# radiocosmology/draco

Measured on AMD Instinct MI355X. Metric: m-modes/sec through MModeTransform+DirtyMapMaker (128-feed, 256-freq), higher is better.
Workload: dtype f64 accumulate; B stored complex128; FFT complex64 (as the reference); 1 GPU; cfg3: 128-feed (379 stacked baselines), 256 freq per GPU (256 in the job), 1024 RA, lmax=mmax=512: MModeTransform.process + DirtyMapMaker.process through the task classes (131328 (m,f) solves + alm2map to nside=256 IQUV maps per GPU and day); parallelism=freq-sharded x1, weak scaling (no collective in the timed region)

## Files before the change

### draco_amd/csrc/dmm_ctx.hip

```cpp
#include <stdio.h>
#include <string.h>

#include "dmm_internal.h"

static thread_local char g_err[512] = "";

int dmm_set_error(int code, const char* fmt, ...) {
  va_list ap;
  va_start(ap, fmt);
  vsnprintf(g_err, sizeof(g_err), fmt, ap);
  va_end(ap);
  return code;
}

static const char* const kProfNames[DMM_PROF_NSLOT] = {"gram", "chol", "tridiag", "ql", "backproj", "band", "chase", "solve", "null"};

static void prof_collect(dmm_ctx* c) {
  for (dmm_prof_span& sp : c->prof_open) {
    float ms = 0.f;
    if (hipEventSynchronize(sp.b) == hipSuccess && hipEventElapsedTime(&ms, sp.a, sp.b) == hipSuccess) {
      c->prof_us[sp.slot] += 1e3 * (double)ms;
      ++c->prof_n[sp.slot];
    }
    (void)hipEventDestroy(sp.a);
// ... 105 lines not shown
  else if (!strcmp(name, "ml_rank_stop")) c->opt_ml_rank_stop = (int)value;
  else if (!strcmp(name, "ml_chase_split")) c->opt_ml_chase_split = (int)value;
  else if (!strcmp(name, "dirty_prio")) c->opt_dirty_prio = (int)value;
  else if (!strcmp(name, "ml_eigen")) c->opt_ml_eigen = (int)value;
  else if (!strcmp(name, "ringmap_variant")) c->opt_ringmap_variant = (int)value;
  else if (!strcmp(name, "ml_reduce")) c->opt_ml_reduce = (int)value;
  else if (!strcmp(name, "gram_stage")) c->opt_gram_stage = (int)value;
  else if (!strcmp(name, "wiener_overlap")) c->opt_wiener_overlap = (int)value;
  else if (!strcmp(name, "ml_workspace_mib")) c->opt_ml_ws_mib = value > 0 ? value : 0;
  else if (!strcmp(name, "regrid_workspace_mib")) c->opt_regrid_ws_mib = value > 0 ? value : 0;
  else if (!strcmp(name, "wiener_workspace_mib")) c->opt_wiener_ws_mib = value > 0 ? value : 0;
  else if (!strcmp(name, "profile")) {
    prof_collect(c);
    for (int k = 0; k < DMM_PROF_NSLOT; ++k) c->prof_us[k] = 0.0, c->prof_n[k] = 0;
    c->opt_profile = value != 0;
  }
  else return dmm_set_error(DMM_E_ARG, "dmm_ctx_set_option: unknown option '%s'", name);
  return DMM_OK;
}

int dmm_ctx_get_counter(dmm_ctx* c, const char* name, int64_t* value) {
  DMM_REQUIRE(c != nullptr && name != nullptr && value != nullptr, "dmm_ctx_get_counter: NULL argument");
  if (!strcmp(name, "ml_tiles_direct")) *value = c->ml_tiles_direct;
  else if (!strcmp(name, "ml_tiles_eigen")) *value = c->ml_tiles_eigen;
  else if (!strcmp(name, "ml_tiles_null")) *value = c->ml_tiles_null;
  else if (!strcmp(name, "ml_tiles_stopped")) *value = c->ml_tiles_stopped;
  else if (!strcmp(name, "ml_gram_cached")) *value = c->ml_gram_cached;
  else if (!strcmp(name, "ml_tiles_basis")) *value = c->ml_tiles_basis;
  else if (!strcmp(name, "ml_stop_cols")) *value = c->ml_stop_cols;
  else if (!strcmp(name, "ml_gram_flops")) *value = c->ml_gram_flops;
  else if (!strcmp(name, "ml_band_bytes")) *value = c->ml_band_bytes;
  else if (!strcmp(name, "ml_tiles_ql_failed")) *value = c->ml_tiles_ql_failed;
  else if (!strcmp(name, "ml_early_chunks")) *value = c->ml_early_chunks;
  else if (!strcmp(name, "ml_two_stage_max_order")) *value = dmm_ml_two_stage_max_order();
  else if (!strcmp(name, "build_ab")) {
#ifdef DMM_AB
    *value = 1;
#else
    *value = 0;
#endif
  }
  else if (!strcmp(name, "opt_ml_eigen")) *value = c->opt_ml_eigen;
  else if (!strcmp(name, "opt_sht_synth_form")) *value = c->opt_sht_synth_form;
  else if (!strncmp(name, "prof_", 5)) {
    const size_t len = strlen(name);
    const bool want_n = len > 7 && !strcmp(name + len - 2, "_n");
    const bool want_us = len > 8 && !strcmp(name + len - 3, "_us");
    int slot = -1;
    for (int k = 0; k < DMM_PROF_NSLOT; ++k) {
      const size_t nl = strlen(kProfNames[k]);
      if (!strncmp(name + 5, kProfNames[k], nl) && name[5 + nl] == '_' && 5 + nl + (want_n ? 2 : 3) == len) slot = k;
    }
    if (slot < 0 || !(want_n || want_us)) return dmm_set_error(DMM_E_ARG, "dmm_ctx_get_counter: unknown counter '%s'", name);
    prof_collect(c);
    *value = want_n ? c->prof_n[slot] : (int64_t)(c->prof_us[slot] + 0.5);
  }
  else return dmm_set_error(DMM_E_ARG, "dmm_ctx_get_counter: unknown counter '%s'", name);
  return DMM_OK;
}

int dmm_ctx_set_ml_basis(dmm_ctx* c, void* U, double* sigma, int32_t* rank, int64_t nslots, int rmax, int build) {
  DMM_REQUIRE(c != nullptr, "dmm_ctx_set_ml_basis: ctx is NULL");
  DMM_REQUIRE(U == nullptr || (sigma != nullptr && rank != nullptr && nslots > 0 && rmax >= 64 && rmax % 64 == 0),
              "dmm_ctx_set_ml_basis: a basis needs sigma, rank, a slot count and rmax a multiple of 64");
  c->ml_bs_U = (double2*)U;
  c->ml_bs_sigma = U ? sigma : nullptr;
// ... 65 lines not shown
```

### draco_amd/csrc/dmm_internal.h

```cpp
#pragma once
#include <hip/hip_runtime.h>
#include <stdint.h>
#include <stdarg.h>
#include <map>
#include <vector>

#include "draco_amd.h"

template <typename T2>
struct dmm_fft_tables {
  int n = 0;
  int M = 0;
  T2* tw = nullptr;
  T2* chirp = nullptr;
  T2* bfilt = nullptr;
};

enum dmm_prof_slot { DMM_PROF_GRAM = 0, DMM_PROF_CHOL, DMM_PROF_TRIDIAG, DMM_PROF_QL, DMM_PROF_BACKPROJ, DMM_PROF_BAND, DMM_PROF_CHASE, DMM_PROF_SOLVE, DMM_PROF_NULL, DMM_PROF_NSLOT };
struct dmm_prof_span {
  hipEvent_t a, b;
  int slot;
};

struct dmm_ctx {
  int device = 0;
  hipStream_t stream = nullptr;
  hipEvent_t ev0 = nullptr, ev1 = nullptr;
  hipStream_t aux_stream = nullptr;
  hipStream_t aux_stream_b = nullptr;
  hipEvent_t aux_ev[4] = {nullptr, nullptr, nullptr, nullptr};
  int* aux_pinned = nullptr;
  size_t aux_pinned_n = 0;
  int num_cu = 256;
  std::map<int, dmm_fft_tables<float2>> fft_f32;
  std::map<int, dmm_fft_tables<double2>> fft_f64;
  std::map<int64_t, void*> sht;
  int opt_dirty_variant = 0;
  int opt_grid_mult = 0;
  int opt_dirty_prio = 0;
  int opt_dirty_static = 0;
  int opt_dirty_nofill = 0;
  int opt_project_grid_mult = 0;
  int opt_project_variant = 0;
  int opt_ml_inner_sweeps = 0, opt_ml_outer_sweeps = 0;
  int opt_sht_variant = 0;
  int opt_sht_synth_form = 0;
  int opt_ml_eigen = 0;
  int64_t opt_regrid_ws_mib = 0;
  int64_t opt_ml_ws_mib = 0, opt_wiener_ws_mib = 0;
  int opt_ml_shortcut = 0;
  int ml_probe_every = 8;
  double ml_pass_rate = 1.0;
  int opt_ml_null = 0;
  int64_t ml_gram_flops = 0, ml_band_bytes = 0;
  int64_t ml_tiles_null = 0;
  int opt_ml_chase_split = 0;
  int opt_ml_rank_stop = 0;
  int64_t ml_order_hist[17] = {};
  int64_t ml_tiles_stopped = 0, ml_stop_cols = 0;
  int64_t ml_tiles_direct = 0, ml_tiles_eigen = 0;
  int64_t ml_tiles_ql_failed = 0;
  int opt_ringmap_variant = 0;
  int opt_wiener_overlap = 1;
  int opt_gram_stage = 0;
  int opt_ml_reduce = 0;
  double2* ml_bs_U = nullptr;
  double* ml_bs_sigma = nullptr;
  int32_t* ml_bs_rank = nullptr;
  int64_t ml_bs_slots = 0;
// ... 125 lines not shown
```

### draco_amd/csrc/sht.hip

```cpp
#include "sht_common.h"
#include "sht_legendre.h"
#include "sht_rings.h"

namespace {

int get_geom(dmm_ctx* ctx, int nside, int lmax, int mmax, ShtGeom* out) {
  const int64_t key = ((int64_t)nside << 40) | ((int64_t)lmax << 20) | (int64_t)mmax;
  auto it = ctx->sht.find(key);
  const int nring = 4 * nside - 1;
  const size_t nd = (size_t)3 * nring + (mmax + 1);
  const size_t bytes = nd * sizeof(double) + (size_t)nring * sizeof(int64_t) + (size_t)nring * sizeof(int);
  const size_t coef_ofs = (bytes + 63) / 64 * 64;
  const size_t coef_rows = (size_t)coef_row0(mmax + 1, lmax);
  int blue_rmax = 0;
  std::vector<int64_t> bf_off(1, 0);
  int64_t bf_total = 0;
  for (int ir = 1; ir < nside && blue_len(ir) <= kMaxBlue; ++ir) {
    bf_off.push_back(bf_total);
    bf_total += blue_len(ir);
    blue_rmax = ir;
  }
  const size_t bfo_ofs = coef_ofs + coef_rows * sizeof(Coef);
  const size_t bf_ofs = (bfo_ofs + bf_off.size() * sizeof(int64_t) + 63) / 64 * 64;
  const size_t phase_ofs = (bf_ofs + (size_t)bf_total * sizeof(double2) + 63) / 64 * 64;
  int tw_len = kMaxBlue;
  while (tw_len < 4 * nside) tw_len <<= 1;
  const size_t tw_ofs = phase_ofs + (size_t)nring * (mmax + 1) * sizeof(double2);
  const size_t chirp_ofs = tw_ofs + (size_t)(tw_len / 2) * sizeof(double2);
  const size_t total = chirp_ofs + (size_t)2 * blue_rmax * (blue_rmax + 1) * sizeof(double2);
  if (it == ctx->sht.end()) {
    std::vector<unsigned char> h(bytes);
    double* z = reinterpret_cast<double*>(h.data());
    double* sth = z + nring;
    double* phi0 = sth + nring;
    double* lfac = phi0 + nring;
    int64_t* start = reinterpret_cast<int64_t*>(lfac + (mmax + 1));
    int* nphi = reinterpret_cast<int*>(start + nring);
    const int64_t npix = 12LL * nside * nside, ncap = 2LL * nside * (nside - 1);
    for (int k = 0; k < nring; ++k) {
      const int64_t ir = k + 1;
      if (ir < nside) {
        z[k] = 1.0 - (double)(ir * ir) / (3.0 * nside * (double)nside);
        nphi[k] = (int)(4 * ir);
        phi0[k] = M_PI / (4.0 * ir);
        start[k] = 2 * ir * (ir - 1);
      } else if (ir <= 3LL * nside) {
        z[k] = (2.0 * nside - ir) * 2.0 / (3.0 * nside);
        nphi[k] = 4 * nside;
        phi0[k] = ((ir - nside + 1) & 1) * M_PI / (4.0 * nside);
        start[k] = ncap + (ir - nside) * 4LL * nside;
      } else {
        const int64_t ip = 4LL * nside - ir;
        z[k] = -(1.0 - (double)(ip * ip) / (3.0 * nside * (double)nside));
        nphi[k] = (int)(4 * ip);
        phi0[k] = M_PI / (4.0 * ip);
        start[k] = npix - 2 * ip * (ip + 1);
      }
      sth[k] = sqrt((1.0 - z[k]) * (1.0 + z[k]));
    }
    double acc = 0.5 * (log2(1.0) - log2(4.0 * M_PI));
    lfac[0] = acc;
    double prod = 0.0;
    for (int m = 1; m <= mmax; ++m) {
      prod += log2((2.0 * m - 1.0) / (2.0 * m));
      lfac[m] = 0.5 * (log2(2.0 * m + 1.0) - log2(4.0 * M_PI) + prod);
    }
    void* d = nullptr;
    DMM_HIP(hipMalloc(&d, total));
    unsigned char* db = static_cast<unsigned char*>(d);
    hipError_t e = hipMemcpy(d, h.data(), bytes, hipMemcpyHostToDevice);
    if (e == hipSuccess) e = hipMemcpy(db + bfo_ofs, bf_off.data(), bf_off.size() * sizeof(int64_t), hipMemcpyHostToDevice);
    if (e == hipSuccess) {
      hipLaunchKernelGGL(k_fill_coef, dim3(mmax + 1), dim3(256), 0, ctx->stream, reinterpret_cast<Coef*>(db + coef_ofs), lmax);
      e = hipGetLastError();
    }
    if (e == hipSuccess && blue_rmax > 0) {
      const int Mmax = blue_len(blue_rmax);
      const size_t lds = ((size_t)Mmax + 1 + Mmax / 2) * sizeof(double2);
      e = hipFuncSetAttribute((const void*)k_build_bfilt, hipFuncAttributeMaxDynamicSharedMemorySize, (int)lds);
      if (e == hipSuccess) {
        hipLaunchKernelGGL(k_build_bfilt, dim3(blue_rmax), dim3(kFftThreads), lds, ctx->stream,
                           reinterpret_cast<double2*>(db + bf_ofs), reinterpret_cast<const int64_t*>(db + bfo_ofs));
        e = hipGetLastError();
      }
    }
    if (e == hipSuccess) {
      hipLaunchKernelGGL(k_fill_ring_tables, dim3(nring + 1 + blue_rmax), dim3(256), 0, ctx->stream,
                         reinterpret_cast<const double*>(db) + 2 * (size_t)nring , nring, mmax,
                         reinterpret_cast<double2*>(db + phase_ofs), reinterpret_cast<double2*>(db + tw_ofs), tw_len,
                         reinterpret_cast<double2*>(db + chirp_ofs));
      e = hipGetLastError();
    }
    if (e != hipSuccess) {
      (void)hipFree(d);
      return dmm_set_error((int)e, "sht geometry upload: %s", hipGetErrorString(e));
    }
    it = ctx->sht.emplace(key, d).first;
  }
  ShtGeom g;
  g.nside = nside;
  g.lmax = lmax;
  g.mmax = mmax;
  g.nring = nring;
  g.block = it->second;
  g.z = reinterpret_cast<double*>(g.block);
  g.sth = g.z + nring;
  g.phi0 = g.sth + nring;
  g.lfac = g.phi0 + nring;
  g.start = reinterpret_cast<int64_t*>(g.lfac + (mmax + 1));
  g.nphi = reinterpret_cast<int*>(g.start + nring);
  unsigned char* gb = static_cast<unsigned char*>(g.block);
  g.coef = reinterpret_cast<double*>(gb + coef_ofs);
  g.bf_off = reinterpret_cast<int64_t*>(gb + bfo_ofs);
  g.bfilt = reinterpret_cast<double2*>(gb + bf_ofs);
  g.blue_rmax = blue_rmax;
  g.phase = reinterpret_cast<double2*>(gb + phase_ofs);
  g.tw = reinterpret_cast<double2*>(gb + tw_ofs);
  g.tw_len = tw_len;
  g.chirp = reinterpret_cast<double2*>(gb + chirp_ofs);
  *out = g;
  return DMM_OK;
}

int check_args(const char* who, dmm_ctx* ctx, const void* a, const void* b, int nfreq, int npol, int lmax, int mmax,
               int nside) {
  DMM_REQUIRE(ctx && a && b, "%s: NULL argument", who);
  DMM_REQUIRE(nfreq >= 1 && lmax >= 0 && mmax >= 0 && mmax <= lmax, "%s: bad sizes nfreq=%d lmax=%d mmax=%d", who, nfreq, lmax, mmax);
  DMM_REQUIRE(npol == 1 || npol == 4, "%s: npol must be 1 or 4 (got %d)", who, npol);
  DMM_REQUIRE(nside >= 1 && (nside & (nside - 1)) == 0 && nside <= 8192, "%s: nside must be a power of two (got %d)", who, nside);
  return DMM_OK;
}

size_t chunk_freqs(int nfreq, int npol, int nring, int mmax) {
  const size_t grp = npol == 4 ? kSynF : 1;
  const size_t per_f = (size_t)npol * nring * (mmax + 1) * sizeof(double2);
  size_t nf = ((size_t)1 << 30) / per_f / grp * grp;
  if (nf < grp) nf = grp;
  if (nf > (size_t)nfreq) nf = nfreq;
  const size_t nchunk = ((size_t)nfreq + nf - 1) / nf;
  const size_t c = ((size_t)nfreq + nchunk - 1) / nchunk;
  return c < (size_t)nfreq ? (c + grp - 1) / grp * grp : c;
}

size_t coef_scratch_bytes(size_t nfc, int npol, int nring, int mmax) {
  const size_t nfs = npol == 4 ? (nfc + kSynF - 1) / kSynF * kSynF : nfc;
  return nfs * npol * nring * (size_t)(mmax + 1) * sizeof(double2);
}

struct ClassLaunch {
  RingClass rc;
  int nblock;
  int nphi_max;
  bool blue;
};

std::vector<ClassLaunch> ring_classes(const ShtGeom& g) {
  std::vector<ClassLaunch> out;
  ClassLaunch b;
  b.rc.belt = 1;
  b.rc.r_lo = b.rc.r_hi = 0;
  b.rc.M = 4 * g.nside;
  b.rc.logM = 0;
  while ((1 << b.rc.logM) < b.rc.M) ++b.rc.logM;
  b.nblock = 2 * g.nside + 1;
  b.nphi_max = 4 * g.nside;
  b.blue = false;
  out.push_back(b);
  for (int ir = 1; ir < g.nside;) {
    const int M = blue_len(ir);
    int hi = ir;
    while (hi + 1 < g.nside && blue_len(hi + 1) == M) ++hi;
    ClassLaunch c;
    c.rc.belt = 0;
    c.rc.r_lo = ir;
    c.rc.r_hi = hi;
    c.rc.M = M;
    c.rc.logM = 0;
    while ((1 << c.rc.logM) < M) ++c.rc.logM;
    c.nblock = 2 * (hi - ir + 1);
    c.nphi_max = 4 * hi;
    c.blue = true;
    out.push_back(c);
    ir = hi + 1;
  }
  return out;
}

size_t ring_fft_lds(const ShtGeom& g, const ClassLaunch& c, int nrow, int force_direct) {
  if (force_direct) return 0;
  if (c.blue && c.rc.r_hi > g.blue_rmax) return 0;
  const size_t lds = ((size_t)nrow * (c.rc.M + 1) + c.rc.M / 2 + (c.blue ? c.nphi_max : 0)) * sizeof(double2);
  return lds <= 160 * 1024 ? lds : 0;
}

size_t ring_synth_lds(const ShtGeom& g, const ClassLaunch& c, int nb, bool stage_all, int force_direct) {
  if (force_direct) return 0;
  if (c.blue && c.rc.r_hi > g.blue_rmax) return 0;
  const int nm = g.mmax + 1;
  const bool staged = stage_all || 4 * (c.blue ? c.rc.r_lo : g.nside) < nm;
  const size_t lds = ((size_t)nb * (c.rc.M + 1) + c.rc.M / 2 + (c.blue ? c.nphi_max : 0) + (staged ? (size_t)nb * 2 * nm : 0)) *
                     sizeof(double2);
  return lds <= 160 * 1024 ? lds : 0;
}

using RingKernel = void (*)(RingParams, RingClass);

int launch_ring(RingKernel kern, dim3 grid, int threads, size_t lds, hipStream_t st, const RingParams& rp, const RingClass& rc) {
  if (lds > 160 * 1024) return dmm_set_error(DMM_E_UNSUPPORTED, "SHT ring stage needs %zu bytes of LDS (nside too large)", lds);
  DMM_HIP(hipFuncSetAttribute((const void*)kern, hipFuncAttributeMaxDynamicSharedMemorySize, (int)lds));
  hipLaunchKernelGGL(kern, grid, dim3(threads), lds, st, rp, rc);
  DMM_HIP(hipGetLastError());
  return DMM_OK;
}

RingParams ring_params(const ShtGeom& g, int nf, int npol, double2* b, double* map, const double* map_ref) {
  RingParams rp;
  rp.g = g;
  rp.nf = nf;
  rp.npol = npol;
  rp.b = b;
  rp.map = map;
  rp.map_ref = map_ref;
  rp.npix = 12LL * g.nside * g.nside;
  rp.stage_all = 0;
  return rp;
}

#define DMM_BY_NPOL(npol, f, ...) ((npol) == 4 ? f<4>(__VA_ARGS__) : f<1>(__VA_ARGS__))

template <int NPOL>
int synth_chunk(dmm_ctx* ctx, const ShtGeom& g, const double2* alm, int n_m, int nf, double2* b, double* map) {
  LegParams lp;
  lp.g = g;
  lp.nf = nf;
  lp.npol = NPOL;
  lp.n_m = n_m;
  lp.alm = alm;
  lp.b = b;
  if (NPOL == 4 && !(ctx->opt_sht_variant & 8)) {
    const int npair = (g.nring + 1) / 2;
    const int nrc = (npair + kThreads - 1) / kThreads;
    const int nx = g.mmax + 1;
    const int64_t col_bytes = (int64_t)4 * n_m * (g.lmax + 1) * (int64_t)sizeof(double2);
    const bool fits8 = 2 * kLegF * col_bytes < ((int64_t)1 << 32), fits4 = kLegF * col_bytes < ((int64_t)1 << 32);
    if ((ctx->opt_sht_variant & 64) || ctx->opt_sht_synth_form == 1 || !fits4) {
      const int nz = (nf + kLegF - 1) / kLegF;
      hipLaunchKernelGGL(k_leg_synth_mfma, dim3(nx, nrc, nz), dim3(kThreads), 0, ctx->stream, lp);
    } else if ((ctx->opt_sht_variant & 128) || !fits8) {
      const int nz = (nf + kLegF - 1) / kLegF;
      hipLaunchKernelGGL(k_leg_synth_mfma2<1>, dim3(nx, nrc, nz), dim3(kThreads), 0, ctx->stream, lp);
    } else {
      const int nz = (nf + 2 * kLegF - 1) / (2 * kLegF);
      hipLaunchKernelGGL(k_leg_synth_mfma2<2>, dim3(nx, nrc, nz), dim3(kThreads), 0, ctx->stream, lp);
    }
  } else {
    hipLaunchKernelGGL(k_leg_synth<NPOL>, dim3(g.mmax + 1, nf), dim3(kThreads), 0, ctx->stream, lp);
  }
  DMM_HIP(hipGetLastError());
  RingParams rp = ring_params(g, nf, NPOL, b, map, nullptr);
  constexpr int KF = NPOL == 4 ? kSynF : 1;
  const dim3 per_ring((nf + KF - 1) / KF, NPOL == 4 ? 2 : 1);
  const int force_direct = ctx->opt_sht_variant & 4;
  constexpr int N2 = NPOL == 4 ? 2 : 1, N4 = NPOL == 4 ? 4 : 1;
  static const RingKernel fft_kernel[3][2] = {{k_ring_synth_fft<NPOL, 1, false>, k_ring_synth_fft<NPOL, 1, true>},
                                              {k_ring_synth_fft<NPOL, N2, false>, k_ring_synth_fft<NPOL, N2, true>},
                                              {k_ring_synth_fft<NPOL, N4, false>, k_ring_synth_fft<NPOL, N4, true>}};
  for (const ClassLaunch& c : ring_classes(g)) {
    int nb = 0;
    size_t lds = 0;
    rp.stage_all = 0;
    for (int tier = 0; tier < 3 && nb == 0; ++tier)
      for (int b = KF; b >= 1 && nb == 0; b >>= 1) {
        const size_t l = ring_synth_lds(g, c, b, tier == 0, force_direct);
        if (l != 0 && l <= (tier < 2 ? (size_t)80 * 1024 : (size_t)160 * 1024)) nb = b, lds = l, rp.stage_all = tier == 0;
      }
    const int rc = nb == 0 ? launch_ring(k_ring_synth<NPOL>, dim3(c.nblock, nf), kThreads, (size_t)NPOL * (g.mmax + 1) * sizeof(double2),
                                         ctx->stream, rp, c.rc)
                           : launch_ring(fft_kernel[nb >> 1][c.blue], dim3(c.nblock, per_ring.x, per_ring.y), kFftThreads, lds,
                                         ctx->stream, rp, c.rc);
    if (rc) return rc;
  }
  return DMM_OK;
}

template <int NPOL>
int anal_chunk(dmm_ctx* ctx, const ShtGeom& g, const double* map, int n_m, int nf, double2* b, double2* alm, int accumulate,
               const double* map_ref = nullptr) {
  const RingParams rp = ring_params(g, nf, NPOL, b, const_cast<double*>(map), map_ref);
  constexpr int NROWS = NPOL == 4 ? 2 : 1;
  const int force_direct = ctx->opt_sht_variant & 4;
  static const RingKernel fft_kernel[2][2] = {{k_ring_anal_fft<NPOL, 1, false>, k_ring_anal_fft<NPOL, 1, true>},
                                              {k_ring_anal_fft<NPOL, NROWS, false>, k_ring_anal_fft<NPOL, NROWS, true>}};
  for (const ClassLaunch& c : ring_classes(g)) {
    const size_t lds2 = ring_fft_lds(g, c, NROWS, force_direct), lds1 = ring_fft_lds(g, c, 1, force_direct);
    const bool both = NROWS == 2 && lds2 != 0 && lds2 <= 80 * 1024;
    const int rc = lds1 == 0 ? launch_ring(k_ring_anal<NPOL>, dim3(c.nblock, nf), kThreads, (size_t)NPOL * c.nphi_max * sizeof(double),
                                           ctx->stream, rp, c.rc)
                             : launch_ring(fft_kernel[both][c.blue], dim3(c.nblock, nf, both ? 1 : NROWS), kFftThreads,
                                           both ? lds2 : lds1, ctx->stream, rp, c.rc);
    if (rc) return rc;
  }
  LegAnalParams lp;
  lp.g = g;
  lp.nf = nf;
  lp.npol = NPOL;
  lp.n_m = n_m;
  lp.b = b;
  lp.alm = alm;
  lp.accumulate = accumulate;
  if (NPOL == 4 && !(ctx->opt_sht_variant & 8)) {
    hipLaunchKernelGGL(k_leg_anal_mfma, dim3(g.mmax + 1, (nf + kLegF - 1) / kLegF), dim3(kThreads), 0, ctx->stream, lp);
    DMM_HIP(hipGetLastError());
    return DMM_OK;
  }
  constexpr int NV = NPOL == 4 ? 8 : 2;
  const size_t lds2 = (size_t)(g.lmax + 1) * NV * sizeof(double) + (size_t)2 * (kThreads / 64) * kAnalBatch * NV * sizeof(double);
  DMM_HIP(hipFuncSetAttribute((const void*)k_leg_anal<NPOL>, hipFuncAttributeMaxDynamicSharedMemorySize, (int)lds2));
  hipLaunchKernelGGL(k_leg_anal<NPOL>, dim3(g.mmax + 1, nf), dim3(kThreads), lds2, ctx->stream, lp);
  DMM_HIP(hipGetLastError());
  return DMM_OK;
}

}

extern "C" {

int dmm_alm2map(dmm_ctx* ctx, const void* alm, int nfreq, int npol, int lmax, int mmax, int nside, double* map) {
  int rc = check_args("dmm_alm2map", ctx, alm, map, nfreq, npol, lmax, mmax, nside);
  if (rc) return rc;
  DMM_HIP(hipSetDevice(ctx->device));
  ShtGeom g;
  rc = get_geom(ctx, nside, lmax, mmax, &g);
  if (rc) return rc;
  const size_t nfc = chunk_freqs(nfreq, npol, g.nring, mmax);
  void* scratch = nullptr;
  rc = dmm_get_scratch(ctx, coef_scratch_bytes(nfc, npol, g.nring, mmax), &scratch);
  if (rc) return rc;
  const int64_t npix = 12LL * nside * nside;
  const int n_m = mmax + 1;
  for (int f0 = 0; f0 < nfreq; f0 += (int)nfc) {
    const int nf = (int)((size_t)(nfreq - f0) < nfc ? (size_t)(nfreq - f0) : nfc);
    const double2* a = (const double2*)alm + (int64_t)f0 * npol * n_m * (lmax + 1);
    double* mp = map + (int64_t)f0 * npol * npix;
    rc = DMM_BY_NPOL(npol, synth_chunk, ctx, g, a, n_m, nf, (double2*)scratch, mp);
    if (rc) return rc;
  }
  return DMM_OK;
}

int dmm_map2alm(dmm_ctx* ctx, const double* map, int nfreq, int npol, int lmax, int mmax, int nside, int niter,
                void* alm) {
  int rc = check_args("dmm_map2alm", ctx, map, alm, nfreq, npol, lmax, mmax, nside);
  if (rc) return rc;
  DMM_REQUIRE(niter >= 0 && niter <= 64, "dmm_map2alm: niter=%d out of range", niter);
  if ((size_t)npol * 4 * nside * sizeof(double) > 150 * 1024)
    return dmm_set_error(DMM_E_UNSUPPORTED, "dmm_map2alm: nside=%d too large for the in-LDS ring stage", nside);
  DMM_HIP(hipSetDevice(ctx->device));
  ShtGeom g;
  rc = get_geom(ctx, nside, lmax, mmax, &g);
  if (rc) return rc;
  const int64_t npix = 12LL * nside * nside;
  size_t nfc = chunk_freqs(nfreq, npol, g.nring, mmax);
  const size_t b_bytes = coef_scratch_bytes(nfc, npol, g.nring, mmax);
  const size_t r_bytes = niter > 0 ? nfc * npol * (size_t)npix * sizeof(double) : 0;
  void* scratch = nullptr;
  rc = dmm_get_scratch(ctx, b_bytes + r_bytes, &scratch);
  if (rc) return rc;
  double2* b = (double2*)scratch;
  double* resid = (double*)((unsigned char*)scratch + b_bytes);
  const int n_m = mmax + 1;
  for (int f0 = 0; f0 < nfreq; f0 += (int)nfc) {
    const int nf = (int)((size_t)(nfreq - f0) < nfc ? (size_t)(nfreq - f0) : nfc);
    double2* a = (double2*)alm + (int64_t)f0 * npol * n_m * (lmax + 1);
    const double* mp = map + (int64_t)f0 * npol * npix;
    rc = DMM_BY_NPOL(npol, anal_chunk, ctx, g, mp, n_m, nf, b, a, 0);
    if (rc) return rc;
    for (int it = 0; it < niter; ++it) {
      rc = DMM_BY_NPOL(npol, synth_chunk, ctx, g, a, n_m, nf, b, resid);
      if (rc) return rc;
      rc = DMM_BY_NPOL(npol, anal_chunk, ctx, g, resid, n_m, nf, b, a, 1, mp);
      if (rc) return rc;
    }
  }
  return DMM_OK;
}

}
```

### draco_amd/csrc/sht_common.h

```cpp
#pragma once
#include <math.h>

#include <vector>

#include "dmm_internal.h"
#include "fft_lds.h"

namespace {


constexpr int kThreads = 256;
constexpr double kBig = 0x1p+740, kSmallStep = 0x1p-800;

constexpr int kSynF = 4;
constexpr int kSynRow = kSynF * 4;
__host__ __device__ __forceinline__ int64_t syn4_at(int f, int m, int ring, int r, int nring, int nm) {
  return ((((int64_t)(f / kSynF) * 2 + r) * nring + ring) * nm + m) * kSynRow + 4 * (f % kSynF);
}
__host__ __device__ __forceinline__ int syn4_slot(int pol) { return pol == 1 || pol == 2 ? 1 : 0; }

struct ShtGeom {
  int nside, lmax, mmax, nring;
  double* z;
  double* sth;
  double* phi0;
  int* nphi;
  int64_t* start;
  double* lfac;
  double* coef;
  double2* bfilt;
  int64_t* bf_off;
  int blue_rmax;
  double2* phase;
  double2* tw;
  int tw_len;
  double2* chirp;
  void* block;
};

__host__ __device__ __forceinline__ int64_t coef_row0(int m, int lmax) {
  return (int64_t)m * (lmax + 1) - (int64_t)m * (m - 1) / 2;
}

struct LegParams {
  ShtGeom g;
  int nf;
  int npol;
  int n_m;
  const double2* alm;
  double2* b;
};

struct Coef {
  double ra, rb;
  double c1, c2;
  double cd, c3;
  double c4, pad;
};

typedef const __attribute__((address_space(4))) double* kptr;
// ... 20 lines not shown
    Coef q;
    const double dl = (double)l, dm = (double)m;
    const double A = sqrt((dl * dl - dm * dm) / (4.0 * dl * dl - 1.0));
    const double l1 = dl - 1.0;
    const double Ap = (l > m) ? sqrt((l1 * l1 - dm * dm) / (4.0 * l1 * l1 - 1.0)) : 0.0;
    q.ra = (l > m) ? 1.0 / A : 0.0;
    q.rb = (l > m) ? Ap / A : 0.0;
    const double c = (l >= 2) ? 2.0 / sqrt((dl - 1.0) * dl * (dl + 1.0) * (dl + 2.0)) : 0.0;
    const double d = (l >= 1) ? sqrt((2.0 * dl + 1.0) / (2.0 * dl - 1.0) * (dl * dl - dm * dm)) : 0.0;
    q.c1 = c * (dl - dm * dm);
    q.c2 = c * 0.5 * dl * (dl - 1.0);
    q.cd = c * d;
    q.c3 = c * dm * (dl - 1.0);
    q.c4 = c * dm * d;
    q.pad = 0.0;
    coef[l - m] = q;
  }
}
static_assert(sizeof(Coef) == 64, "Coef row");

__device__ __forceinline__ void lam_start(double lfac_m, int m, double sth, double& v, int& nsc) {
  const double lg = lfac_m + (double)m * log2(sth);
  nsc = 0;
  if (lg < -700.0) nsc = (int)ceil((-lg - 700.0) / 800.0);
  v = exp2(lg + 800.0 * (double)nsc);
  if (m & 1) v = -v;
}

__device__ __forceinline__ bool ring_skips_m(int m, int lmax, double sth) {
  const double ofs = fmax(100.0, 0.01 * (double)lmax);
  return (double)m > (double)lmax * sth + ofs + 2.0;
}

}
```

### draco_amd/csrc/sht_legendre.h

```cpp
#pragma once
#include "sht_common.h"

namespace {

typedef double v4d __attribute__((ext_vector_type(4)));

struct LegRing {
  double x, inv_s2, xs2, lam, lam_prev;
  int nsc;
};

__device__ __forceinline__ LegRing leg_ring_start(const ShtGeom& g, int m, int r, int npair) {
  LegRing R = {0.0, 0.0, 0.0, 0.0, 0.0, -1};
  if (r < npair) {
    const double sth = g.sth[r];
    R.x = g.z[r];
    R.inv_s2 = 1.0 / (sth * sth);
    R.xs2 = R.x * R.inv_s2;
    if (!ring_skips_m(m, g.lmax, sth)) lam_start(g.lfac[m], m, sth, R.lam, R.nsc);
  }
  return R;
}

__device__ __forceinline__ void leg_advance(LegRing& R, double ra, double rb) {
// ... 103 lines not shown
      const int kc = k < nl ? k : nl - 1;
      __builtin_amdgcn_s_waitcnt(0xc07f);
      Ops o;
      o.q = load_coef(coef + 8 * kc);
      o.aT = load_c(a[0] + 2 * kc);
      o.aE = o.aB = o.aV = make_double2(0.0, 0.0);
      if (NPOL == 4) {
        o.aE = load_c(a[NPOL > 1 ? 1 : 0] + 2 * kc);
        o.aB = load_c(a[NPOL > 1 ? 2 : 0] + 2 * kc);
        o.aV = load_c(a[NPOL > 1 ? 3 : 0] + 2 * kc);
      }
      return o;
    };
    Ops cur = fetch(0);
    for (int k = 0; k < nl; k += 2) {
      Ops nxt = fetch(k + 1);
#pragma unroll
      for (int t = 0; t < NR; ++t) step(R[t], S[t], cur.q, cur.aT, cur.aE, cur.aB, cur.aV, k == 0, true);
      if (k + 1 >= nl) break;
      cur = fetch(k + 2);
#pragma unroll
      for (int t = 0; t < NR; ++t) step(R[t], S[t], nxt.q, nxt.aT, nxt.aE, nxt.aB, nxt.aV, false, false);
    }
#pragma unroll
    for (int t = 0; t < NR; ++t) {
      const int r = r0 + t * kThreads + threadIdx.x;
      if (r >= npair) continue;
      const int rs = nring - 1 - r;
      const Sums& g = S[t];
      auto val = [&](double2 s, double2 an, double sgn) { return make_double2(s.x + sgn * an.x, s.y + sgn * an.y); };
      if (NPOL == 1) {
        p.b[((int64_t)f * nring + r) * mstride + m] = val(g.Ts, g.Ta, 1.0);
        if (rs != r) p.b[((int64_t)f * nring + rs) * mstride + m] = val(g.Ts, g.Ta, -1.0);
      } else {
        double* bout = reinterpret_cast<double*>(p.b);
        auto put = [&](int ring, int tr, double2 v0, double2 v1) {
          double* q = bout + syn4_at(f, m, ring, tr, nring, (int)mstride);
          *reinterpret_cast<double2*>(q) = make_double2(v0.x, v1.x);
          *reinterpret_cast<double2*>(q + 2) = make_double2(v0.y, v1.y);
        };
        put(r, 0, val(g.Ts, g.Ta, 1.0), val(g.Qs, g.Qa, 1.0));
        put(r, 1, val(g.Vs, g.Va, 1.0), val(g.Us, g.Ua, 1.0));
        if (rs != r) {
          put(rs, 0, val(g.Ts, g.Ta, -1.0), val(g.Qs, g.Qa, -1.0));
          put(rs, 1, val(g.Vs, g.Va, -1.0), val(g.Us, g.Ua, -1.0));
        }
      }
    }
  }
}

constexpr int kLegL = 8, kLegF = 4, kLegPitch = 72;
static_assert(kLegF == kSynF, "a frequency group of the MFMA columns is one group of the synthesis scratch");

template <class TileRing>
__device__ __forceinline__ void leg_store_syn4(const LegParams& p, int f, int m, const LegCol& col, int kq, const v4d (&acc)[4][4],
                                               TileRing tile0) {
  const int nring = p.g.nring, npair = (nring + 1) / 2, nm = p.g.mmax + 1;
  double* bout = reinterpret_cast<double*>(p.b) + 2 * col.comp;
#pragma unroll
  for (int t = 0; t < 4; ++t)
#pragma unroll
    for (int reg = 0; reg < 4; ++reg) {
      const int rr = tile0(t) + kq + 4 * reg;
      if (rr >= npair) continue;
      const int rs = nring - 1 - rr;
      const double tv = acc[t][0][reg], tva = acc[t][1][reg], qu = acc[t][2][reg], qua = acc[t][3][reg];
      *reinterpret_cast<double2*>(bout + syn4_at(f, m, rr, col.c >> 1, nring, nm)) = make_double2(tv + tva, qu + qua);
      if (rs != rr) *reinterpret_cast<double2*>(bout + syn4_at(f, m, rs, col.c >> 1, nring, nm)) = make_double2(tv - tva, qu - qua);
    }
}

__global__ __launch_bounds__(kThreads, 2) void k_leg_synth_mfma(LegParams p) {
  __shared__ double slab[kThreads / 64][3][kLegL][kLegPitch];
  const int m = blockIdx.x, rc = blockIdx.y, f0 = blockIdx.z * kLegF;
  const int lmax = p.g.lmax, nl = lmax - m + 1;
  const int lane = threadIdx.x & 63, wave = threadIdx.x >> 6;
  double(*sl)[kLegL][kLegPitch] = slab[wave];

  LegRing R = leg_ring_start(p.g, m, rc * kThreads + threadIdx.x, (p.g.nring + 1) / 2);
  const bool wave_live = __any(R.nsc >= 0);

  const int li = lane & 15, kq = lane >> 4;
  const LegCol col = leg_col(lane);
  const int f = f0 + col.fi;
  const bool fok = f < p.nf;
  auto colptr = [&](int pol, int comp) {
    return reinterpret_cast<const double*>(p.alm + (((int64_t)(fok ? f : 0) * 4 + pol) * p.n_m + m) * (lmax + 1) + m) + comp;
  };
  const double* pTV = colptr(col.polTV, col.comp);
  const double* p1 = colptr(col.pol1, col.comp);
  const double* p2 = colptr(col.pol2, col.comp ^ 1);
  const double s2 = col.f2neg ? -1.0 : 1.0;

  v4d acc[4][4];
#pragma unroll
  for (int t = 0; t < 4; ++t)
#pragma unroll
// ... 563 lines not shown
```

### draco_amd/csrc/sht_rings.h

```cpp
#pragma once
#include "sht_common.h"

namespace {

struct RingParams {
  ShtGeom g;
  int nf, npol;
  double2* b;
  double* map;
  int64_t npix;
  const double* map_ref;
  int stage_all;
};

struct RingClass {
  int belt;
  int r_lo, r_hi;
  int M, logM;
};
constexpr int kMinBlue = 256, kMaxBlue = 4096;

__host__ __device__ __forceinline__ int blue_len(int ir) {
  int M = kMinBlue;
  while (M < 8 * ir - 1) M <<= 1;
  return M;
}

__device__ __forceinline__ int class_ring(const RingClass& rc, const ShtGeom& g, int i) {
  if (rc.belt) return g.nside - 1 + i;
  const int ir = rc.r_lo + (i >> 1);
  return (i & 1) ? g.nring - ir : ir - 1;
}

template <int NPOL>
__global__ __launch_bounds__(kThreads) void k_ring_synth(RingParams p, RingClass rc) {
  extern __shared__ __align__(16) unsigned char smem[];
  double2* c = reinterpret_cast<double2*>(smem);
  const int ring = class_ring(rc, p.g, blockIdx.x);
  const int f = blockIdx.y;
  const int nm = p.g.mmax + 1;
  const double phi0 = p.g.phi0[ring];
  const int nphi = p.g.nphi[ring];
  for (int idx = threadIdx.x; idx < NPOL * nm; idx += kThreads) {
    const int pol = idx / nm, m = idx - pol * nm;
    double2 v;
    if (NPOL == 1) {
      v = p.b[((int64_t)f * p.g.nring + ring) * nm + m];
    } else {
      const double* q = reinterpret_cast<const double*>(p.b) + syn4_at(f, m, ring, pol >> 1, p.g.nring, nm) + syn4_slot(pol);
      v = make_double2(q[0], q[2]);
    }
    double sn, cs;
    sincos((double)m * phi0, &sn, &cs);
    const double fac = m == 0 ? 1.0 : 2.0;
    c[idx] = make_double2(fac * (v.x * cs - v.y * sn), fac * (v.x * sn + v.y * cs));
  }
  __syncthreads();
  const int64_t base = p.g.start[ring];
  for (int j = threadIdx.x; j < nphi; j += kThreads) {
    double sn, cs;
    sincospi(2.0 * (double)j / (double)nphi, &sn, &cs);
    double pr = 1.0, pi_ = 0.0;
    double acc[NPOL];
#pragma unroll
    for (int q = 0; q < NPOL; ++q) acc[q] = 0.0;
    for (int m = 0; m < nm; ++m) {
#pragma unroll
      for (int q = 0; q < NPOL; ++q) {
        const double2 cm = c[q * nm + m];
        acc[q] = fma(cm.x, pr, fma(-cm.y, pi_, acc[q]));
      }
      const double nr = pr * cs - pi_ * sn;
      pi_ = fma(pr, sn, pi_ * cs);
      pr = nr;
    }
#pragma unroll
    for (int q = 0; q < NPOL; ++q) p.map[((int64_t)f * NPOL + q) * p.npix + base + j] = acc[q];
  }
}

constexpr int kFftThreads = 256;

struct RingLds {
  dmm_fft::C<double>* buf;
  dmm_fft::C<double>* tw;
  dmm_fft::C<double>* chirp;
};

template <int NROW, bool BLUE>
__device__ __forceinline__ RingLds ring_lds(unsigned char* smem, const ShtGeom& g, int N, int M) {
  RingLds l;
  l.buf = reinterpret_cast<dmm_fft::C<double>*>(smem);
  l.tw = l.buf + NROW * (M + 1);
  l.chirp = l.tw + (M >> 1);
  const int stride = g.tw_len / M;
  for (int k = threadIdx.x; k < (M >> 1); k += kFftThreads) {
    const double2 t = g.tw[k * stride];
    l.tw[k] = {t.x, t.y};
  }
// ... 42 lines not shown
  if (BLUE) dmm_fft::bluestein_convolve<double, kFftThreads>(l.buf, l.tw, bfilt, NROW, M, logM, P, true);
  else dmm_fft::fft_dif8<double, kFftThreads>(l.buf, l.tw, NROW, M, logM, P);
}

template <bool BLUE>
__device__ __forceinline__ dmm_fft::C<double> ring_dft_at(const RingLds& l, int r, int k, int M, int logM) {
  if (BLUE) return dmm_fft::cmul<double>(l.buf[r * (M + 1) + k], l.chirp[k]);
  return l.buf[r * (M + 1) + dmm_fft::bitrev(k, logM)];
}

template <int NPOL, int NB, bool BLUE>
__global__ __launch_bounds__(kFftThreads) void k_ring_synth_fft(RingParams p, RingClass rc) {
  using dmm_fft::C;
  constexpr int KF = NPOL == 4 ? kSynF : 1;
  static_assert(KF % NB == 0, "passes of NB transforms");
  extern __shared__ __align__(16) unsigned char smem[];
  const int ring = class_ring(rc, p.g, blockIdx.x), r = NPOL == 4 ? (int)blockIdx.z : 0;
  const int f0 = KF * blockIdx.y, nfb = min(KF, p.nf - f0);
  const int n = p.g.nphi[ring], M = rc.M, P = M + 1;
  const RingLds l = ring_lds<NB, BLUE>(smem, p.g, n, M);
  if (BLUE) __syncthreads();
  const int nm = p.g.mmax + 1;
  const double2* phase = p.g.phase + (int64_t)ring * nm;
  auto load = [&](int fi, int m, double2& va, double2& vb) {
    if (NPOL == 1) {
      va = p.b[((int64_t)(f0 + fi) * p.g.nring + ring) * nm + m];
    } else {
      const double* q = reinterpret_cast<const double*>(p.b) + syn4_at(f0 + fi, m, ring, r, p.g.nring, nm);
      const double2 re = *reinterpret_cast<const double2*>(q), im = *reinterpret_cast<const double2*>(q + 2);
      va = r == 0 ? make_double2(re.x, im.x) : make_double2(re.y, im.y);
      vb = r == 0 ? make_double2(re.y, im.y) : make_double2(re.x, im.x);
    }
  };
  const bool staged = p.stage_all || n < nm;
  C<double>* rot = l.chirp + (BLUE ? 4 * rc.r_hi : 0);
  const double2* bfilt = BLUE ? p.g.bfilt + p.g.bf_off[rc.belt ? 0 : rc.r_lo + ((int)blockIdx.x >> 1)] : nullptr;
  const int64_t base = p.g.start[ring];
  for (int fb = 0; fb < nfb; fb += NB) {
    if (fb > 0) __syncthreads();
    if (staged) {
      for (int q = threadIdx.x; q < NB * nm; q += kFftThreads) {
        const int m = q / NB, j = q - m * NB;
        C<double> a = {0.0, 0.0}, b = {0.0, 0.0};
        if (fb + j < nfb) {
          const double2 ph = phase[m];
          const double cs = ph.x, sn = ph.y;
          double2 va, vb;
          load(fb + j, m, va, vb);
          a = {va.x * cs - va.y * sn, va.x * sn + va.y * cs};
          if (NPOL == 4) b = {vb.x * cs - vb.y * sn, vb.x * sn + vb.y * cs};
          if (m == 0) a.y = b.y = 0.0;
        }
        rot[(j * 2 + 0) * nm + m] = a;
        rot[(j * 2 + 1) * nm + m] = b;
      }
      __syncthreads();
    }
    for (int k = threadIdx.x; k < M; k += kFftThreads) {
      double zr[NB], zi[NB];
#pragma unroll
      for (int j = 0; j < NB; ++j) zr[j] = zi[j] = 0.0;
      if (k < n && staged) {
        for (int m = k; m < nm; m += n) {
#pragma unroll
          for (int j = 0; j < NB; ++j) {
            const C<double> a = rot[(j * 2 + 0) * nm + m], b = rot[(j * 2 + 1) * nm + m];
            zr[j] += a.x - b.y;
            zi[j] += a.y + b.x;
          }
        }
        for (int m = (k == 0 ? n : n - k); m < nm; m += n) {
#pragma unroll
          for (int j = 0; j < NB; ++j) {
            const C<double> a = rot[(j * 2 + 0) * nm + m], b = rot[(j * 2 + 1) * nm + m];
            zr[j] += a.x + b.y;
            zi[j] += b.x - a.y;
          }
        }
      } else if (k < n) {
        for (int m = k; m < nm; m += n) {
          const double2 ph = phase[m];
          const double cs = ph.x, sn = ph.y;
#pragma unroll
          for (int j = 0; j < NB; ++j) {
            if (fb + j >= nfb) continue;
            double2 va, vb;
            load(fb + j, m, va, vb);
            double ar = va.x * cs - va.y * sn, ai = va.x * sn + va.y * cs;
            double br = 0.0, bi = 0.0;
            if (NPOL == 4) {
              br = vb.x * cs - vb.y * sn;
              bi = vb.x * sn + vb.y * cs;
            }
            if (m == 0) ai = bi = 0.0;
            zr[j] += ar - bi;
            zi[j] += ai + br;
          }
        }
        for (int m = (k == 0 ? n : n - k); m < nm; m += n) {
          const double2 ph = phase[m];
          const double cs = ph.x, sn = ph.y;
#pragma unroll
          for (int j = 0; j < NB; ++j) {
            if (fb + j >= nfb) continue;
            double2 va, vb;
            load(fb + j, m, va, vb);
            const double ar = va.x * cs - va.y * sn, ai = va.x * sn + va.y * cs;
            double br = 0.0, bi = 0.0;
            if (NPOL == 4) {
              br = vb.x * cs - vb.y * sn;
              bi = vb.x * sn + vb.y * cs;
            }
            zr[j] += ar + bi;
            zi[j] += br - ai;
          }
        }
      }
#pragma unroll
      for (int j = 0; j < NB; ++j) {
        C<double> v = {zr[j], -zi[j]};
        if (BLUE && k < n) v = dmm_fft::cmul<double>(v, l.chirp[k]);
        l.buf[j * P + k] = v;
      }
    }
    __syncthreads();
    ring_dft<NB, BLUE>(l, bfilt, M, rc.logM);
    for (int j = threadIdx.x; j < n; j += kFftThreads) {
#pragma unroll
      for (int jj = 0; jj < NB; ++jj) {
        if (fb + jj >= nfb) continue;
        const int64_t f = f0 + fb + jj;
        const C<double> y = ring_dft_at<BLUE>(l, jj, j, M, rc.logM);
// ... 131 lines not shown
```

Before: 2070 m-modes/s.

## Truncate per-ring m range in SHT synthesis using precomputed mlim table

Computes a per-ring maximum m (mlim) on the device from the existing ring_skips_m criterion, caches it per geometry, and uses it to bound the Legendre output writes, the ring synthesis loops and the staged rotation buffer. Polar rings where high m contribute negligibly then skip the loads, rotations and fold-ins for those m. LDS for the staged buffer is sized by the per-class max nrot, which may let more blocks fit per CU. Adds a one-time device sync and counters, and relies on the Legendre stage leaving unwritten slots unused.

```diff
diff --git a/draco_amd/csrc/dmm_ctx.hip b/draco_amd/csrc/dmm_ctx.hip
--- a/draco_amd/csrc/dmm_ctx.hip
+++ b/draco_amd/csrc/dmm_ctx.hip
@@ -161,6 +161,8 @@
   else if (!strcmp(name, "ml_band_bytes")) *value = c->ml_band_bytes;
   else if (!strcmp(name, "ml_tiles_ql_failed")) *value = c->ml_tiles_ql_failed;
   else if (!strcmp(name, "ml_early_chunks")) *value = c->ml_early_chunks;
+  else if (!strcmp(name, "sht_skipped_slots")) *value = c->sht_skipped_slots;
+  else if (!strcmp(name, "sht_mlim_mismatch")) *value = c->sht_mlim_mismatch;
   else if (!strcmp(name, "ml_two_stage_max_order")) *value = dmm_ml_two_stage_max_order();
   else if (!strcmp(name, "build_ab")) {
 #ifdef DMM_AB
diff --git a/draco_amd/csrc/dmm_internal.h b/draco_amd/csrc/dmm_internal.h
--- a/draco_amd/csrc/dmm_internal.h
+++ b/draco_amd/csrc/dmm_internal.h
@@ -35,6 +35,8 @@
   std::map<int, dmm_fft_tables<float2>> fft_f32;
   std::map<int, dmm_fft_tables<double2>> fft_f64;
   std::map<int64_t, void*> sht;
+  std::map<int64_t, std::vector<int>> sht_mlim;
+  int64_t sht_skipped_slots = 0, sht_mlim_mismatch = 0;
   int opt_dirty_variant = 0;
   int opt_grid_mult = 0;
   int opt_dirty_prio = 0;
diff --git a/draco_amd/csrc/sht.hip b/draco_amd/csrc/sht.hip
--- a/draco_amd/csrc/sht.hip
+++ b/draco_amd/csrc/sht.hip
@@ -1,15 +1,17 @@
+#include <algorithm>
+
 #include "sht_common.h"
 #include "sht_legendre.h"
 #include "sht_rings.h"
 
 namespace {
 
-int get_geom(dmm_ctx* ctx, int nside, int lmax, int mmax, ShtGeom* out) {
+int get_geom(dmm_ctx* ctx, int nside, int lmax, int mmax, ShtGeom* out, const int** mlim_host) {
   const int64_t key = ((int64_t)nside << 40) | ((int64_t)lmax << 20) | (int64_t)mmax;
   auto it = ctx->sht.find(key);
   const int nring = 4 * nside - 1;
   const size_t nd = (size_t)3 * nring + (mmax + 1);
-  const size_t bytes = nd * sizeof(double) + (size_t)nring * sizeof(int64_t) + (size_t)nring * sizeof(int);
+  const size_t bytes = nd * sizeof(double) + (size_t)nring * sizeof(int64_t) + 2 * sizeof(unsigned long long) + (size_t)2 * nring * sizeof(int);
   const size_t coef_ofs = (bytes + 63) / 64 * 64;
   const size_t coef_rows = (size_t)coef_row0(mmax + 1, lmax);
   int blue_rmax = 0;
@@ -35,7 +37,7 @@
     double* phi0 = sth + nring;
     double* lfac = phi0 + nring;
     int64_t* start = reinterpret_cast<int64_t*>(lfac + (mmax + 1));
-    int* nphi = reinterpret_cast<int*>(start + nring);
+    int* nphi = reinterpret_cast<int*>(start + nring + 2);
     const int64_t npix = 12LL * nside * nside, ncap = 2LL * nside * (nside - 1);
     for (int k = 0; k < nring; ++k) {
       const int64_t ir = k + 1;
@@ -91,10 +93,25 @@
                          reinterpret_cast<double2*>(db + chirp_ofs));
       e = hipGetLastError();
     }
+    std::vector<int> mlim_h(nring);
+    unsigned long long stats[2] = {0, 0};
+    if (e == hipSuccess) {
+      unsigned long long* dstats = reinterpret_cast<unsigned long long*>(db + nd * sizeof(double) + (size_t)nring * sizeof(int64_t));
+      int* dmlim = reinterpret_cast<int*>(dstats + 2) + nring;
+      hipLaunchKernelGGL(k_fill_mlim, dim3(nring), dim3(256), 0, ctx->stream, reinterpret_cast<const double*>(db) + nring , lmax,
+                         mmax, dmlim, dstats);
+      e = hipGetLastError();
+      if (e == hipSuccess) e = hipMemcpyAsync(mlim_h.data(), dmlim, (size_t)nring * sizeof(int), hipMemcpyDeviceToHost, ctx->stream);
+      if (e == hipSuccess) e = hipMemcpyAsync(stats, dstats, sizeof(stats), hipMemcpyDeviceToHost, ctx->stream);
+      if (e == hipSuccess) e = hipStreamSynchronize(ctx->stream);
+    }
     if (e != hipSuccess) {
       (void)hipFree(d);
       return dmm_set_error((int)e, "sht geometry upload: %s", hipGetErrorString(e));
     }
+    ctx->sht_skipped_slots += (int64_t)stats[0];
+    ctx->sht_mlim_mismatch += (int64_t)stats[1];
+    ctx->sht_mlim[key] = std::move(mlim_h);
     it = ctx->sht.emplace(key, d).first;
   }
   ShtGeom g;
@@ -108,7 +125,9 @@
   g.phi0 = g.sth + nring;
   g.lfac = g.phi0 + nring;
   g.start = reinterpret_cast<int64_t*>(g.lfac + (mmax + 1));
-  g.nphi = reinterpret_cast<int*>(g.start + nring);
+  g.nphi = reinterpret_cast<int*>(g.start + nring + 2);
+  g.mlim = g.nphi + nring;
+  *mlim_host = ctx->sht_mlim[key].data();
   unsigned char* gb = static_cast<unsigned char*>(g.block);
   g.coef = reinterpret_cast<double*>(gb + coef_ofs);
   g.bf_off = reinterpret_cast<int64_t*>(gb + bfo_ofs);
@@ -154,8 +173,13 @@
   bool blue;
 };
 
-std::vector<ClassLaunch> ring_classes(const ShtGeom& g) {
+std::vector<ClassLaunch> ring_classes(const ShtGeom& g, const int* mlim = nullptr) {
   std::vector<ClassLaunch> out;
+  auto nrot_of = [&](int first, int last) {
+    int v = 0;
+    for (int k = first; mlim && k <= last; ++k) v = std::max(v, std::max(mlim[k], mlim[g.nring - 1 - k]) + 1);
+    return v;
+  };
   ClassLaunch b;
   b.rc.belt = 1;
   b.rc.r_lo = b.rc.r_hi = 0;
@@ -165,6 +189,7 @@
   b.nblock = 2 * g.nside + 1;
   b.nphi_max = 4 * g.nside;
   b.blue = false;
+  b.rc.nrot = nrot_of(g.nside - 1, 2 * g.nside - 1);
   out.push_back(b);
   for (int ir = 1; ir < g.nside;) {
     const int M = blue_len(ir);
@@ -180,6 +205,7 @@
     c.nblock = 2 * (hi - ir + 1);
     c.nphi_max = 4 * hi;
     c.blue = true;
+    c.rc.nrot = nrot_of(ir - 1, hi - 1);
     out.push_back(c);
     ir = hi + 1;
   }
@@ -193,12 +219,12 @@
   return lds <= 160 * 1024 ? lds : 0;
 }
 
-size_t ring_synth_lds(const ShtGeom& g, const ClassLaunch& c, int nb, bool stage_all, int force_direct) {
+size_t ring_synth_lds(const ShtGeom& g, const ClassLaunch& c, int nb, bool stage_all, int nrot, int force_direct) {
   if (force_direct) return 0;
   if (c.blue && c.rc.r_hi > g.blue_rmax) return 0;
   const int nm = g.mmax + 1;
   const bool staged = stage_all || 4 * (c.blue ? c.rc.r_lo : g.nside) < nm;
-  const size_t lds = ((size_t)nb * (c.rc.M + 1) + c.rc.M / 2 + (c.blue ? c.nphi_max : 0) + (staged ? (size_t)nb * 2 * nm : 0)) *
+  const size_t lds = ((size_t)nb * (c.rc.M + 1) + c.rc.M / 2 + (c.blue ? c.nphi_max : 0) + (staged ? (size_t)nb * 2 * nrot : 0)) *
                      sizeof(double2);
   return lds <= 160 * 1024 ? lds : 0;
 }
@@ -229,7 +255,7 @@
 #define DMM_BY_NPOL(npol, f, ...) ((npol) == 4 ? f<4>(__VA_ARGS__) : f<1>(__VA_ARGS__))
 
 template <int NPOL>
-int synth_chunk(dmm_ctx* ctx, const ShtGeom& g, const double2* alm, int n_m, int nf, double2* b, double* map) {
+int synth_chunk(dmm_ctx* ctx, const ShtGeom& g, const int* mlim, const double2* alm, int n_m, int nf, double2* b, double* map) {
   LegParams lp;
   lp.g = g;
   lp.nf = nf;
@@ -265,15 +291,16 @@
   static const RingKernel fft_kernel[3][2] = {{k_ring_synth_fft<NPOL, 1, false>, k_ring_synth_fft<NPOL, 1, true>},
                                               {k_ring_synth_fft<NPOL, N2, false>, k_ring_synth_fft<NPOL, N2, true>},
                                               {k_ring_synth_fft<NPOL, N4, false>, k_ring_synth_fft<NPOL, N4, true>}};
-  for (const ClassLaunch& c : ring_classes(g)) {
+  for (const ClassLaunch& c : ring_classes(g, mlim)) {
     int nb = 0;
     size_t lds = 0;
     rp.stage_all = 0;
     for (int tier = 0; tier < 3 && nb == 0; ++tier)
       for (int b = KF; b >= 1 && nb == 0; b >>= 1) {
-        const size_t l = ring_synth_lds(g, c, b, tier == 0, force_direct);
-        if (l != 0 && l <= (tier < 2 ? (size_t)80 * 1024 : (size_t)160 * 1024)) nb = b, lds = l, rp.stage_all = tier == 0;
+        const size_t l = ring_synth_lds(g, c, b, tier == 0, g.mmax + 1, force_direct);
+        if (l != 0 && l <= (tier < 2 ? (size_t)80 * 1024 : (size_t)160 * 1024)) nb = b, rp.stage_all = tier == 0;
       }
+    if (nb) lds = ring_synth_lds(g, c, nb, rp.stage_all != 0, c.rc.nrot, force_direct);
     const int rc = nb == 0 ? launch_ring(k_ring_synth<NPOL>, dim3(c.nblock, nf), kThreads, (size_t)NPOL * (g.mmax + 1) * sizeof(double2),
                                          ctx->stream, rp, c.rc)
                            : launch_ring(fft_kernel[nb >> 1][c.blue], dim3(c.nblock, per_ring.x, per_ring.y), kFftThreads, lds,
@@ -330,7 +357,8 @@
   if (rc) return rc;
   DMM_HIP(hipSetDevice(ctx->device));
   ShtGeom g;
-  rc = get_geom(ctx, nside, lmax, mmax, &g);
+  const int* mlim = nullptr;
+  rc = get_geom(ctx, nside, lmax, mmax, &g, &mlim);
   if (rc) return rc;
   const size_t nfc = chunk_freqs(nfreq, npol, g.nring, mmax);
   void* scratch = nullptr;
@@ -342,7 +370,7 @@
     const int nf = (int)((size_t)(nfreq - f0) < nfc ? (size_t)(nfreq - f0) : nfc);
     const double2* a = (const double2*)alm + (int64_t)f0 * npol * n_m * (lmax + 1);
     double* mp = map + (int64_t)f0 * npol * npix;
-    rc = DMM_BY_NPOL(npol, synth_chunk, ctx, g, a, n_m, nf, (double2*)scratch, mp);
+    rc = DMM_BY_NPOL(npol, synth_chunk, ctx, g, mlim, a, n_m, nf, (double2*)scratch, mp);
     if (rc) return rc;
   }
   return DMM_OK;
@@ -357,7 +385,8 @@
     return dmm_set_error(DMM_E_UNSUPPORTED, "dmm_map2alm: nside=%d too large for the in-LDS ring stage", nside);
   DMM_HIP(hipSetDevice(ctx->device));
   ShtGeom g;
-  rc = get_geom(ctx, nside, lmax, mmax, &g);
+  const int* mlim = nullptr;
+  rc = get_geom(ctx, nside, lmax, mmax, &g, &mlim);
   if (rc) return rc;
   const int64_t npix = 12LL * nside * nside;
   size_t nfc = chunk_freqs(nfreq, npol, g.nring, mmax);
@@ -376,7 +405,7 @@
     rc = DMM_BY_NPOL(npol, anal_chunk, ctx, g, mp, n_m, nf, b, a, 0);
     if (rc) return rc;
     for (int it = 0; it < niter; ++it) {
-      rc = DMM_BY_NPOL(npol, synth_chunk, ctx, g, a, n_m, nf, b, resid);
+      rc = DMM_BY_NPOL(npol, synth_chunk, ctx, g, mlim, a, n_m, nf, b, resid);
       if (rc) return rc;
       rc = DMM_BY_NPOL(npol, anal_chunk, ctx, g, resid, n_m, nf, b, a, 1, mp);
       if (rc) return rc;
diff --git a/draco_amd/csrc/sht_common.h b/draco_amd/csrc/sht_common.h
--- a/draco_amd/csrc/sht_common.h
+++ b/draco_amd/csrc/sht_common.h
@@ -26,6 +26,7 @@
   double* phi0;
   int* nphi;
   int64_t* start;
+  int* mlim;
   double* lfac;
   double* coef;
   double2* bfilt;
@@ -112,4 +113,23 @@
   return (double)m > (double)lmax * sth + ofs + 2.0;
 }
 
+__global__ void k_fill_mlim(const double* sth, int lmax, int mmax, int* mlim, unsigned long long* stats) {
+  __shared__ int lim;
+  const int ring = blockIdx.x;
+  const double s = sth[ring];
+  if (threadIdx.x == 0) {
+    int m = mmax;
+    while (m > 0 && ring_skips_m(m, lmax, s)) --m;
+    lim = mlim[ring] = m;
+  }
+  __syncthreads();
+  unsigned long long nskip = 0, nbad = 0;
+  for (int m = threadIdx.x; m <= mmax; m += blockDim.x) {
+    nskip += m > lim;
+    nbad += ring_skips_m(m, lmax, s) != (m > lim);
+  }
+  if (nskip) atomicAdd(&stats[0], nskip);
+  if (nbad) atomicAdd(&stats[1], nbad);
 }
+
+}
diff --git a/draco_amd/csrc/sht_legendre.h b/draco_amd/csrc/sht_legendre.h
--- a/draco_amd/csrc/sht_legendre.h
+++ b/draco_amd/csrc/sht_legendre.h
@@ -159,7 +159,7 @@
       if (NPOL == 1) {
         p.b[((int64_t)f * nring + r) * mstride + m] = val(g.Ts, g.Ta, 1.0);
         if (rs != r) p.b[((int64_t)f * nring + rs) * mstride + m] = val(g.Ts, g.Ta, -1.0);
-      } else {
+      } else if (m <= p.g.mlim[r]) {
         double* bout = reinterpret_cast<double*>(p.b);
         auto put = [&](int ring, int tr, double2 v0, double2 v1) {
           double* q = bout + syn4_at(f, m, ring, tr, nring, (int)mstride);
@@ -190,7 +190,7 @@
 #pragma unroll
     for (int reg = 0; reg < 4; ++reg) {
       const int rr = tile0(t) + kq + 4 * reg;
-      if (rr >= npair) continue;
+      if (rr >= npair || m > p.g.mlim[rr]) continue;
       const int rs = nring - 1 - rr;
       const double tv = acc[t][0][reg], tva = acc[t][1][reg], qu = acc[t][2][reg], qua = acc[t][3][reg];
       *reinterpret_cast<double2*>(bout + syn4_at(f, m, rr, col.c >> 1, nring, nm)) = make_double2(tv + tva, qu + qua);
diff --git a/draco_amd/csrc/sht_rings.h b/draco_amd/csrc/sht_rings.h
--- a/draco_amd/csrc/sht_rings.h
+++ b/draco_amd/csrc/sht_rings.h
@@ -17,6 +17,7 @@
   int belt;
   int r_lo, r_hi;
   int M, logM;
+  int nrot;
 };
 constexpr int kMinBlue = 256, kMaxBlue = 4096;
 
@@ -41,8 +42,9 @@
   const int nm = p.g.mmax + 1;
   const double phi0 = p.g.phi0[ring];
   const int nphi = p.g.nphi[ring];
-  for (int idx = threadIdx.x; idx < NPOL * nm; idx += kThreads) {
-    const int pol = idx / nm, m = idx - pol * nm;
+  const int nl = p.g.mlim[ring] + 1;
+  for (int idx = threadIdx.x; idx < NPOL * nl; idx += kThreads) {
+    const int pol = idx / nl, m = idx - pol * nl;
     double2 v;
     if (NPOL == 1) {
       v = p.b[((int64_t)f * p.g.nring + ring) * nm + m];
@@ -53,7 +55,7 @@
     double sn, cs;
     sincos((double)m * phi0, &sn, &cs);
     const double fac = m == 0 ? 1.0 : 2.0;
-    c[idx] = make_double2(fac * (v.x * cs - v.y * sn), fac * (v.x * sn + v.y * cs));
+    c[pol * nm + m] = make_double2(fac * (v.x * cs - v.y * sn), fac * (v.x * sn + v.y * cs));
   }
   __syncthreads();
   const int64_t base = p.g.start[ring];
@@ -64,7 +66,7 @@
     double acc[NPOL];
 #pragma unroll
     for (int q = 0; q < NPOL; ++q) acc[q] = 0.0;
-    for (int m = 0; m < nm; ++m) {
+    for (int m = 0; m < nl; ++m) {
 #pragma unroll
       for (int q = 0; q < NPOL; ++q) {
         const double2 cm = c[q * nm + m];
@@ -173,14 +175,16 @@
       vb = r == 0 ? make_double2(re.y, im.y) : make_double2(re.x, im.x);
     }
   };
+  const int nl = p.g.mlim[ring] + 1;
   const bool staged = p.stage_all || n < nm;
+  const int nr = rc.nrot;
   C<double>* rot = l.chirp + (BLUE ? 4 * rc.r_hi : 0);
   const double2* bfilt = BLUE ? p.g.bfilt + p.g.bf_off[rc.belt ? 0 : rc.r_lo + ((int)blockIdx.x >> 1)] : nullptr;
   const int64_t base = p.g.start[ring];
   for (int fb = 0; fb < nfb; fb += NB) {
     if (fb > 0) __syncthreads();
     if (staged) {
-      for (int q = threadIdx.x; q < NB * nm; q += kFftThreads) {
+      for (int q = threadIdx.x; q < NB * nl; q += kFftThreads) {
         const int m = q / NB, j = q - m * NB;
         C<double> a = {0.0, 0.0}, b = {0.0, 0.0};
         if (fb + j < nfb) {
@@ -192,8 +196,8 @@
           if (NPOL == 4) b = {vb.x * cs - vb.y * sn, vb.x * sn + vb.y * cs};
           if (m == 0) a.y = b.y = 0.0;
         }
-        rot[(j * 2 + 0) * nm + m] = a;
-        rot[(j * 2 + 1) * nm + m] = b;
+        rot[(j * 2 + 0) * nr + m] = a;
+        rot[(j * 2 + 1) * nr + m] = b;
       }
       __syncthreads();
     }
@@ -202,24 +206,24 @@
 #pragma unroll
       for (int j = 0; j < NB; ++j) zr[j] = zi[j] = 0.0;
       if (k < n && staged) {
-        for (int m = k; m < nm; m += n) {
+        for (int m = k; m < nl; m += n) {
 #pragma unroll
           for (int j = 0; j < NB; ++j) {
-            const C<double> a = rot[(j * 2 + 0) * nm + m], b = rot[(j * 2 + 1) * nm + m];
+            const C<double> a = rot[(j * 2 + 0) * nr + m], b = rot[(j * 2 + 1) * nr + m];
             zr[j] += a.x - b.y;
             zi[j] += a.y + b.x;
           }
         }
-        for (int m = (k == 0 ? n : n - k); m < nm; m += n) {
+        for (int m = (k == 0 ? n : n - k); m < nl; m += n) {
 #pragma unroll
           for (int j = 0; j < NB; ++j) {
-            const C<double> a = rot[(j * 2 + 0) * nm + m], b = rot[(j * 2 + 1) * nm + m];
+            const C<double> a = rot[(j * 2 + 0) * nr + m], b = rot[(j * 2 + 1) * nr + m];
             zr[j] += a.x + b.y;
             zi[j] += b.x - a.y;
           }
         }
       } else if (k < n) {
-        for (int m = k; m < nm; m += n) {
+        for (int m = k; m < nl; m += n) {
           const double2 ph = phase[m];
           const double cs = ph.x, sn = ph.y;
 #pragma unroll
@@ -238,7 +242,7 @@
             zi[j] += ai + br;
           }
         }
-        for (int m = (k == 0 ? n : n - k); m < nm; m += n) {
+        for (int m = (k == 0 ? n : n - k); m < nl; m += n) {
           const double2 ph = phase[m];
           const double cs = ph.x, sn = ph.y;
 #pragma unroll
```

Result: no change. 2052 m-modes/s (median of 2 runs) (-0.9%).
